# arkworks-rs/circom-compat

Hardware: AMD Instinct MI355X
Metric: Groth16 constraints/sec (BN254) (higher is better)
Workload: dtype int32x9 (29-bit limbs of 254-bit Montgomery integers); 1 GPU; synthetic squaring-chain R1CS, 2^22-2 constraints, BN254, full prove (witness map + 4 G1 MSM + 1 G2 MSM + finalize), trapdoor key minted on GPU; log2_domain=22, num_constraints=4194302, n_vars=4194304, parallelism=single-gpu

## Files before the change

### circom_compat_amd/csrc/api.hip

```cpp
#include "../../include/g16_amd.h"

#include <stddef.h>
#include <stdlib.h>

#include <algorithm>
#include <mutex>

#include "ctx.h"

using namespace g16;

static_assert(offsetof(g16::ProofSums, B1) == sizeof(g16::G1XYZZ29) && offsetof(g16::ProofSums, L) == 2 * sizeof(g16::G1XYZZ29),
              "ProofSums must keep A, B1, L adjacent (batched reduction writes them as an array)");
static_assert(G16_PARTIAL_BYTES == g16::FIN_PARTIAL_BYTES, "partial record size out of sync");

namespace {
std::mutex g_err_mu;
std::string g_create_error;
}


namespace {

g16_status fail(g16_ctx* ctx, g16_status code, const std::string& msg) {
  if (ctx) ctx->err = msg;
  else {
    std::lock_guard<std::mutex> g(g_err_mu);
    g_create_error = msg;
  }
  return code;
}

template <class Fn>
g16_status guarded(g16_ctx* ctx, Fn fn) {
  try {
    if (ctx) G16_HIP(hipSetDevice(ctx->device));
    return fn();
  } catch (const HipError& e) {
    return fail(ctx, G16_ERR_HIP, e.what());
  } catch (const std::bad_alloc&) {
    return fail(ctx, G16_ERR_INTERNAL, "host allocation failed");
  } catch (const std::exception& e) {
    const bool dom = std::string(e.what()).find("PolynomialDegreeTooLarge") != std::string::npos;
    return fail(ctx, dom ? G16_ERR_DOMAIN_TOO_LARGE : G16_ERR_INTERNAL, e.what());
  }
}

void shard(uint32_t len, int rank, int world, uint32_t* lo, uint32_t* hi) {
  *lo = (uint32_t)((uint64_t)len * rank / world);
  *hi = (uint32_t)((uint64_t)len * (rank + 1) / world);
}

int work1_batch(const MsmConfig& cw, uint32_t wr, bool sharded) {
  return (cw.nb() / wr < (1u << 18) || sharded) ? 3 : 2;
}

size_t msm_state_bytes(const MsmConfig& cw, const MsmConfig& ch, uint32_t lw, uint32_t l_cnt, uint32_t lh,
                       uint32_t wr, bool sharded, bool own_w, bool own_h, bool view_w) {
  size_t b = 0;
  if (view_w) b += MsmSort::view_bytes_for(lw, cw);
  if (own_w) b += (size_t)cw.Pn * ((size_t)lw * (64 * 2 + 128) + (size_t)l_cnt * 64);
  if (own_h) b += (size_t)ch.Pn * lh * 64;
  b += MsmSort::bytes_for(lw, cw) + MsmSort::bytes_for(lh, ch);
  const uint32_t nc_w = ceil_div(cw.B, msm_red_chunk(cw, 1, wr)) * cw.D;
  const uint32_t nc_h = ceil_div(ch.B, msm_red_chunk(ch)) * ch.D;
  const uint32_t slots_w = cw.nb() + cw.max_lanes(), slots_h = ch.nb() + ch.max_lanes();
  b += msm_work_bytes<Fq>(slots_w, nc_w, cw.D, work1_batch(cw, wr, sharded)) + msm_work_bytes<Fq2>(slots_w, nc_w, cw.D, 1) +
       msm_work_bytes<Fq>(slots_h, nc_h, ch.D, 1);
  return b;
}

void plan_msm_configs(const g16_options& o, uint32_t lw, uint32_t l_cnt, uint32_t lh, uint32_t wr, bool sharded,
                      bool own_w, bool own_h, bool view_w, MsmConfig* cw, MsmConfig* ch) {
  if (own_w) *cw = msm_make_config(lw ? lw : 1, o.window_bits, o.planes);
  if (own_h) *ch = msm_make_config(lh ? lh : 1, o.window_bits, o.planes);
  if (o.planes > 0) return;
  size_t fr = 0, tot = 0;
  if (hipMemGetInfo(&fr, &tot) != hipSuccess) return;
  const size_t margin = std::min(((size_t)2 << 30) + fr / 50, fr / 4);
  const size_t budget = fr - margin;
  if (msm_state_bytes(*cw, *ch, lw, l_cnt, lh, wr, sharded, own_w, own_h, view_w) <= budget) return;
  auto layouts = [&](const MsmConfig& full, uint32_t len, bool own) {
    std::vector<MsmConfig> v{full};
    for (int pn = full.Pn - 1; own && pn >= 1; --pn) {
      const MsmConfig c = msm_make_config(len ? len : 1, o.window_bits, pn);
      if (c.Pn != v.back().Pn) v.push_back(c);
    }
    return v;
  };
  const std::vector<MsmConfig> vw = layouts(*cw, lw, own_w), vh = layouts(*ch, lh, own_h);
  long best = -1;
  size_t best_bytes = 0;
  for (const MsmConfig& a : vw)
    for (const MsmConfig& b : vh) {
      const size_t need = msm_state_bytes(a, b, lw, l_cnt, lh, wr, sharded, own_w, own_h, view_w);
      if (need > budget) continue;
      const long score = 5L * a.D + b.D;
      if (best < 0 || score < best || (score == best && need > best_bytes)) {
        best = score;
        best_bytes = need;
        *cw = a;
        *ch = b;
      }
    }
  if (best < 0) {
    if (!own_w && !own_h)
      throw std::runtime_error("the sort and partial-sum state of this ctx does not fit the device memory that is free (" +
                               std::to_string(fr >> 20) + " MiB)");
    throw std::runtime_error("the proving key does not fit this device's memory even with one plane per point (" +
                             std::to_string(fr >> 20) + " MiB free)");
  }
}

inline bool sched_r5() {
  static const bool v = [] { const char* e = getenv("G16_SCHED_R5"); return e && atoi(e) != 0; }();
  return v;
}

void collect_times(g16_ctx* c) {
  if (c->timer.enabled) c->timer.collect(c->st_ms, c->st_cnt);
}

void accumulate_ab(g16_ctx* c, hipStream_t s, StageTimer* tm, bool fixup = true) {
  if (c->ptsA.stride == 2) {
    msm_accumulate_pair<Fq>(c->sort_w, c->ptsA, c->ptsB1, c->work1, 0, s, tm, fixup);
  } else {
    msm_accumulate<Fq>(c->sort_w, c->ptsA, 0, c->work1, 0, s, tm, fixup);
    msm_accumulate<Fq>(c->sort_w, c->ptsB1, 0, c->work1, 1, s, tm, fixup);
  }
}
void fixup_ab(g16_ctx* c, hipStream_t q) {
  StageTimer* tm = c->timer.enabled ? &c->timer : nullptr;
  if (c->ptsA.stride == 2) {
    msm_fixup_pair<Fq>(c->sort_w, c->ptsA, c->ptsB1, c->work1, 0, q, tm);
  } else {
    msm_fixup<Fq>(c->sort_w, c->ptsA, 0, c->work1, 0, q, tm);
    msm_fixup<Fq>(c->sort_w, c->ptsB1, 0, c->work1, 1, q, tm);
  }
}

void enqueue_witness_sort(g16_ctx* c, const Fr* w_dev) {
  hipStream_t s = c->stream;
  StageTimer* tm = c->timer.enabled ? &c->timer : nullptr;
  int id = tm ? tm->begin(ST_MSM_SORT, s) : -1;
  c->sort_w.run(w_dev + 1 + c->w_lo, c->w_hi - c->w_lo, true, s);
  if (tm) tm->end(id, s);
  if (c->sparse_b) {
    hipStream_t v = c->overlap ? c->red : s;
    G16_HIP(hipEventRecord(c->ev_view, s));
    G16_HIP(hipStreamWaitEvent(v, c->ev_view, 0));
    id = tm ? tm->begin(ST_MSM_SORT, v) : -1;
    c->sort_b.run_view(c->sort_w, c->keep_b, v);
    if (tm) tm->end(id, v);
    G16_HIP(hipEventRecord(c->ev_view, v));
  }
}
void wait_for_b_view(g16_ctx* c, hipStream_t s) {
  if (c->sparse_b) G16_HIP(hipStreamWaitEvent(s, c->ev_view, 0));
}

template <class Hook, class Hook2>
void enqueue_witness_msms(g16_ctx* c, const Fr* w_dev, Hook after_ab, Hook2 after_b2, bool sorted = false) {
  hipStream_t s = c->stream;
  StageTimer* tm = c->timer.enabled ? &c->timer : nullptr;
  ProofSums* S = c->sums_dev.p;
  if (!sorted) enqueue_witness_sort(c, w_dev);
  const uint32_t nb_eff = c->cfg_w.nb() / (c->shard_buckets ? (uint32_t)c->world : 1u);
  const bool small = nb_eff < (1u << 18);
  const uint32_t b2_limit = c->world > 1 ? (1u << 18) : (1u << 16);
  const bool b2_off = c->overlap && nb_eff < b2_limit;
  const bool sharded = c->world > 1 || c->dist_wm;
  const bool mid = (nb_eff >= (1u << 15) && small) || (sharded && nb_eff >= (1u << 15));
  if (mid && c->overlap && c->work1.batch >= 3) {
    hipStream_t q = c->red;
    accumulate_ab(c, s, tm, false);
    G16_HIP(hipEventRecord(c->ev_acc[0], s));
    G16_HIP(hipStreamWaitEvent(q, c->ev_acc[0], 0));
    fixup_ab(c, q);
    msm_reduce<Fq>(c->sort_w, c->work1, 0, 2, &S->A, q, tm, true);
    after_ab(q);
    wait_for_b_view(c, s);
    msm_accumulate<Fq2>(c->sort_for_b(), c->ptsB2, 0, c->work2, 0, s, tm);
    G16_HIP(hipEventRecord(c->ev_acc[1], s));
    G16_HIP(hipStreamWaitEvent(q, c->ev_acc[1], 0));
    msm_reduce<Fq2>(c->sort_for_b(), c->work2, 0, 1, &S->B2, q, tm, true);
    const bool r5 = sched_r5();
    hipStream_t ql = r5 ? q : c->side;
    if (!r5) after_b2();
    msm_accumulate<Fq>(c->sort_w, c->ptsL, c->l_idx_min, c->work1, 2, s, tm, false);
    G16_HIP(hipEventRecord(c->ev_acc[2], s));
    G16_HIP(hipStreamWaitEvent(ql, c->ev_acc[2], 0));
    msm_fixup<Fq>(c->sort_w, c->ptsL, c->l_idx_min, c->work1, 2, ql, tm);
    msm_reduce<Fq>(c->sort_w, c->work1, 2, 1, &S->L, ql, tm, true);
    if (r5) after_b2();
    G16_HIP(hipEventRecord(c->ev_b2, q));
    G16_HIP(hipStreamWaitEvent(c->side, c->ev_b2, 0));
    G16_HIP(hipEventRecord(c->ev_side, c->side));
    return;
  }
  if (small && c->work1.batch >= 3) {
    accumulate_ab(c, s, tm);
    msm_accumulate<Fq>(c->sort_w, c->ptsL, c->l_idx_min, c->work1, 2, s, tm);
    msm_reduce<Fq>(c->sort_w, c->work1, 0, 3, &S->A, s, tm);
    after_ab(s);
  } else {
    accumulate_ab(c, s, tm);
    msm_reduce<Fq>(c->sort_w, c->work1, 0, 2, &S->A, s, tm);
    after_ab(s);
    msm_run<Fq>(c->sort_w, c->ptsL, c->l_idx_min, c->work1, &S->L, s, tm);
  }
  wait_for_b_view(c, s);
  msm_accumulate<Fq2>(c->sort_for_b(), c->ptsB2, 0, c->work2, 0, s, tm);
  hipStream_t rs = b2_off ? c->red : s;
  G16_HIP(hipEventRecord(c->ev_b2, s));
  G16_HIP(hipStreamWaitEvent(rs, c->ev_b2, 0));
  msm_reduce<Fq2>(c->sort_for_b(), c->work2, 0, 1, &S->B2, rs, tm);
  G16_HIP(hipEventRecord(c->ev_b2, rs));
  if (rs != c->red) G16_HIP(hipStreamWaitEvent(c->red, c->ev_b2, 0));
  after_b2();
  G16_HIP(hipEventRecord(c->ev_b2, c->red));
  G16_HIP(hipStreamWaitEvent(c->side, c->ev_b2, 0));
  G16_HIP(hipEventRecord(c->ev_side, c->side));
}

void enqueue_h_msm(g16_ctx* c) {
  hipStream_t s = c->stream;
  StageTimer* tm = c->timer.enabled ? &c->timer : nullptr;
  G16_HIP(hipStreamWaitEvent(s, c->ev_h, 0));
  msm_run<Fq>(c->sort_h, c->ptsH, 0, c->workH, &c->sums_dev.p->H, s, tm);
}

template <class Hook, class Hook2>
void run_msms(g16_ctx* c, const Fr* w_dev, Hook after_ab, Hook2 after_b2) {
  hipStream_t s = c->stream, x = c->overlap ? c->aux : c->stream;
  StageTimer* tm = c->timer.enabled ? &c->timer : nullptr;
  const uint32_t nb_eff = c->cfg_w.nb() / (c->shard_buckets ? (uint32_t)c->world : 1u);
  const bool sort_first = !sched_r5() && c->overlap && c->world == 1 && nb_eff >= (1u << 18) && c->n <= (1u << 24);
  if (sort_first) enqueue_witness_sort(c, w_dev);
  G16_HIP(hipEventRecord(c->ev_w, s));
  G16_HIP(hipStreamWaitEvent(x, c->ev_w, 0));
  int id = tm ? tm->begin(ST_WITNESS_MAP, x) : -1;
  c->wm.run(w_dev, c->h_canon.p, nullptr, x);
  if (tm) tm->end(id, x);
  id = tm ? tm->begin(ST_MSM_SORT, x) : -1;
  c->sort_h.run(c->h_canon.p + c->h_lo, c->h_hi - c->h_lo, false, x);
  if (tm) tm->end(id, x);
  G16_HIP(hipEventRecord(c->ev_h, x));
  enqueue_witness_msms(c, w_dev, after_ab, after_b2, sort_first);
  enqueue_h_msm(c);
}

template <class Hook>
void run_msms(g16_ctx* c, const Fr* w_dev, Hook after_ab) {
  run_msms(c, w_dev, after_ab, [] {});
}

void begin_sharded(g16_ctx* c, const uint64_t r[4], const uint64_t s_[4]) {
// ... 392 lines not shown
                                 (const G1Affine*)key->b_g1_query + 1 + c->w_lo, lw, c->cfg_w, s);
      }
      c->ptsB2.init((const G2Affine*)key->b_g2_query + 1 + c->w_lo, lw, c->cfg_w, s);
      c->l_idx_min = l_first - c->w_lo;
      c->ptsL.init((const G1Affine*)key->l_query + (l_first - c->p), l_cnt, c->cfg_w, s);
    }
    c->sort_h.init(lh, c->cfg_h);
    if (lend_h) {
      borrow(c->ptsH, lender->ptsH);
    } else if (c->dist_wm) {
      std::vector<G1Affine> mine(lh);
      const G1Affine* hq = (const G1Affine*)key->h_query;
      for (uint32_t t = 0; t < lh; ++t)
        memcpy((void*)&mine[t], (const uint8_t*)hq + (size_t)c->wd.global_index(t) * sizeof(G1Affine), sizeof(G1Affine));
      c->ptsH.init(mine.data(), lh, c->cfg_h, s);
      G16_HIP(hipStreamSynchronize(s));
    } else {
      c->ptsH.init((const G1Affine*)key->h_query + c->h_lo, lh, c->cfg_h, s);
    }

    {
      const bool can = c->world == 1 && !c->dist_wm && c->has_key;
      if (o.fixed_tables > 0 && !can)
        throw std::runtime_error("fixed_tables: only a single-device proving ctx (world = 1, no distributed witness map) can use them");
      if (lender && lend_h) {
        if (lender->tbl.active && o.fixed_tables >= 0) c->tbl.borrow(lender->tbl);
        else if (o.fixed_tables > 0) throw std::runtime_error("fixed_tables: the donor has no tables to lend");
      } else if (can && !lender && o.fixed_tables >= 0) {
        const size_t need = tbl_bytes((size_t)2 * lw + l_cnt + lh, lw);
        size_t fr = 0, tot = 0;
        G16_HIP(hipMemGetInfo(&fr, &tot));
        const bool fits = need <= fr / 3;
        const bool small = lw <= TBL_MAX_POINTS && lh <= TBL_MAX_POINTS;
        if (o.fixed_tables > 0 && !fits)
          throw std::runtime_error("fixed_tables: the tables need " + std::to_string(need >> 20) + " MiB, more than a third of the free device memory");
        if (o.fixed_tables > 0 || (small && fits)) {
          try {
            c->tbl.build(key->a_query + 64, key->b_g1_query + 64, key->b_g2_query + 128,
                         key->l_query + (size_t)(l_first - c->p) * 64, key->h_query, lw, l_first - c->w_lo, l_cnt, lh, s);
          } catch (const HipError&) {
            if (o.fixed_tables > 0) throw;
            (void)hipGetLastError();
            (void)hipStreamSynchronize(s);
            c->tbl.release();
          }
        }
      }
    }

    {
      const uint32_t nc_w = ceil_div(c->cfg_w.B, msm_red_chunk(c->cfg_w, 1, wr)) * c->cfg_w.D;
      const uint32_t nc_h = ceil_div(c->cfg_h.B, msm_red_chunk(c->cfg_h)) * c->cfg_h.D;
      const uint32_t slots_w = c->cfg_w.nb() + c->cfg_w.max_lanes(), slots_h = c->cfg_h.nb() + c->cfg_h.max_lanes();
      c->work1.init(slots_w, nc_w, c->cfg_w.D, work1_batch(c->cfg_w, wr, sharded));
      c->workH.init(slots_h, nc_h, c->cfg_h.D, 1);
      c->work2.init(slots_w, nc_w, c->cfg_w.D);
    }

    KeyHeaderDev kh;
    memcpy(&kh.alpha1, key->alpha_g1, 64);
    memcpy(&kh.beta1, key->beta_g1, 64);
    memcpy(&kh.delta1, key->delta_g1, 64);
    memcpy(&kh.a0, key->a_query, 64);
    memcpy(&kh.b1_0, key->b_g1_query, 64);
    memcpy(&kh.beta2, key->beta_g2, 128);
    memcpy(&kh.delta2, key->delta_g2, 128);
    memcpy(&kh.b2_0, key->b_g2_query, 128);
    G16_HIP(hipMemcpyAsync(c->key_dev.p, &kh, sizeof kh, hipMemcpyHostToDevice, s));
    G16_HIP(hipMemsetAsync(c->out_dev.p, 0, c->out_dev.bytes(), s));
    G16_HIP(hipMemsetAsync(c->sums_dev.p, 0, sizeof(ProofSums), s));
    G16_HIP(hipMemsetAsync(c->fin_scr.p, 0, sizeof(FinScratch), s));
    fin_build_tables(c->key_dev.p, c->fin_tab.p, s);
    G16_HIP(hipStreamSynchronize(s));
    return G16_OK;
  });
  if (st != G16_OK) {
    if (err) *err = c->err;
    g16_ctx_destroy(c);
    return st;
  }
  *out = c;
  return G16_OK;
}

}

extern "C" {

g16_status g16_ctx_create(const g16_key_desc* key, const g16_csr* a, const g16_csr* b,
                          uint32_t num_constraints, const g16_options* opt, g16_ctx** out) {
  std::string err;
  const g16_status st = ctx_create_impl(key, a, b, num_constraints, opt, nullptr, out, &err);
  if (st != G16_OK) return fail(nullptr, st, err);
  return G16_OK;
}

g16_status g16_ctx_create_sibling(g16_ctx* donor, const g16_key_desc* key, const g16_csr* a, const g16_csr* b,
                                  uint32_t num_constraints, const g16_options* opt, g16_ctx** out) {
  if (!donor) return fail(nullptr, G16_ERR_INVALID, "null argument");
  g16_options o{};
  if (opt) o = *opt;
  o.device = donor->device;
  o.rank = 0;
  o.world = 1;
  o.dist_wm = 0;
  if (donor->multi || donor->share_from || !donor->has_key)
    return fail(nullptr, G16_ERR_INVALID, "sibling: the donor must be a plain single-device proving ctx that owns its planes");
// ... 707 lines not shown
```

### circom_compat_amd/csrc/common.h

```cpp
#pragma once
#include <stdint.h>
#include <stdio.h>
#include <string.h>

#include <stdexcept>
#include <string>
#include <vector>

#ifdef G16_EMU
#include <tuple>
#define G16_LAUNCH(kern, grid, block, smem, stream, ...)                                  \
  do {                                                                                    \
    auto _g16_args = std::make_tuple(__VA_ARGS__);      \
    emu::launch(dim3(grid), dim3(block), (smem), [&]() {                                  \
      std::apply([](auto&&... _a) { kern(_a...); }, _g16_args);                           \
    });                                                                                   \
  } while (0)
#define G16_DYN_SMEM(name) unsigned char* name = emu::dyn_smem
#else
#include <hip/hip_runtime.h>
#define G16_LAUNCH(kern, grid, block, smem, stream, ...) \
  hipLaunchKernelGGL(kern, dim3(grid), dim3(block), (smem), (stream), __VA_ARGS__)
#define G16_DYN_SMEM(name) extern __shared__ __attribute__((aligned(16))) unsigned char name[]
#endif

#include "ec.h"

namespace g16 {

struct HipError : std::runtime_error {
  int code;
  HipError(int c, const std::string& m) : std::runtime_error(m), code(c) {}
};

#define G16_HIP(expr)                                                                         \
  do {                                                                                        \
    hipError_t _e = (expr);                                                                   \
    if (_e != hipSuccess) {                                                                   \
      char _b[512];                                                                           \
      snprintf(_b, sizeof _b, "%s failed: %s (%s:%d)", #expr, hipGetErrorString(_e), __FILE__, \
               __LINE__);                                                                     \
      throw g16::HipError((int)_e, _b);                                                       \
    }                                                                                         \
  } while (0)

static inline uint32_t ceil_div(uint64_t a, uint64_t b) { return (uint32_t)((a + b - 1) / b); }

template <class T>
struct DevBuf {
  T* p = nullptr;
  size_t n = 0;
  DevBuf() = default;
  DevBuf(const DevBuf&) = delete;
  DevBuf& operator=(const DevBuf&) = delete;
  ~DevBuf() { release(); }
  void alloc(size_t count) {
    release();
    n = count;
    if (count) G16_HIP(hipMalloc((void**)&p, count * sizeof(T)));
  }
  void release() {
    if (p) (void)hipFree(p);
    p = nullptr;
    n = 0;
  }
  size_t bytes() const { return n * sizeof(T); }
};

enum Stage {
  ST_WITNESS_MAP = 0,
  ST_MSM_SORT,
  ST_MSM_ACC_G1,
  ST_MSM_ACC_G2,
  ST_MSM_REDUCE,
  ST_FINALIZE,
  ST_MSM_ACC_G1_PAIR,
// ... 58 lines not shown
```

### circom_compat_amd/csrc/msm.h

```cpp
#pragma once
#include <stdlib.h>
#include "common.h"
#include "ec29.h"

namespace g16 {

constexpr int MSM_ACC_THREADS = 128;
#ifdef G16_EMU
constexpr int MSM_ACC_BLOCKS = 48;
constexpr int MSM_ACC_BLOCKS_G2 = 32;
#else
constexpr int MSM_ACC_BLOCKS = 3072;
constexpr int MSM_ACC_BLOCKS_G2 = 2048;
#endif
constexpr int MSM_MIN_SEG = 8;
constexpr int MSM_SMALL_MULTI = 32;
constexpr int MSM_RED_CHUNK = 16;
constexpr uint32_t MSM_IDX_BITS_WIDE = 27, MSM_IDX_BITS_NARROW = 26;

struct MsmConfig {
  int c = 0;
  int W = 0;
  int Pn = 1;
  int D = 0;
// ... 62 lines not shown
  const uint32_t* range_dev() const { return world > 1 ? range.p : nullptr; }

  void init(uint32_t capacity, const MsmConfig& cfg);
  void set_shard(int rank, int world);
  void run(const void* scalars, uint32_t n, bool mont, hipStream_t stream);
  void init_view(uint32_t capacity, const MsmConfig& cfg);
  void release_view() {
    count.release(); offset.release(); cursor.release(); entries.release(); multi_l.release();
    meta.release(); multi_l2.release(); meta2.release(); scan_tmp.release();
    cap = len = 0;
  }
  void run_view(const MsmSort& src, const uint32_t* keep_bits, hipStream_t stream);
  static size_t view_bytes_for(uint32_t capacity, const MsmConfig& cfg) {
    const uint64_t M = (uint64_t)capacity * cfg.W;
    return (size_t)(M * 4 + 3 * ((uint64_t)cfg.nb() + 1) * 4 + 2 * (M / ((uint64_t)MSM_MIN_SEG * MSM_SMALL_MULTI) + 2) * 4 + 4096);
  }
  size_t device_bytes() const;
  static size_t bytes_for(uint32_t capacity, const MsmConfig& cfg);
};

template <class F>
using MsmAcc = XYZZ29<typename Lazy<F>::type>;

template <class F>
struct MsmPoints {
  MsmConfig cfg;
  uint32_t count = 0;
  DevBuf<Affine<F>> pts;
  const Affine<F>* view = nullptr;
  uint32_t stride = 1, off = 0;
  const Affine<F>* data() const { return view ? view : pts.p; }
  void init(const Affine<F>* host_points, uint32_t count, const MsmConfig& cfg, hipStream_t stream);
  static void init_pair(MsmPoints& a, MsmPoints& b, const Affine<F>* host_a, const Affine<F>* host_b,
                        uint32_t count, const MsmConfig& cfg, hipStream_t stream);
  void init_from_device(const Affine<F>* dev_points, uint32_t count, const MsmConfig& cfg,
                        hipStream_t stream);
};

#ifdef G16_EMU
constexpr uint32_t MSM_FIX_CAP = 512;
#else
constexpr uint32_t MSM_FIX_CAP = 2048;
#endif
struct MsmFixList {
  uint32_t count;
  uint32_t overflow;
  uint32_t slot[MSM_FIX_CAP];
  uint32_t entry[MSM_FIX_CAP];
};

template <class F>
struct MsmWork {
  int batch = 1;
  uint32_t slots = 0, ncontrib = 0;
  int sets = 1;
  DevBuf<MsmAcc<F>> partial;
  DevBuf<MsmAcc<F>> contrib;
  DevBuf<MsmAcc<F>> bsum;
  DevBuf<MsmAcc<F>> wsum;
  DevBuf<MsmFixList> fix;
  void init(uint32_t n_slots, uint32_t n_contrib, int max_sets, int batch = 1);
};

template <class F>
inline size_t msm_work_bytes(uint32_t n_slots, uint32_t n_contrib, int max_sets, int batch) {
  return (size_t)batch * ((size_t)n_slots + n_contrib + (size_t)257 * max_sets) * sizeof(MsmAcc<F>) +
         (size_t)batch * sizeof(MsmFixList);
}

template <class F>
void msm_run(const MsmSort& s, const MsmPoints<F>& pts, uint32_t idx_min, MsmWork<F>& work,
             MsmAcc<F>* out_dev, hipStream_t stream, StageTimer* tm = nullptr);
template <class F>
void msm_accumulate(const MsmSort& s, const MsmPoints<F>& pts, uint32_t idx_min, MsmWork<F>& work,
                    int slot, hipStream_t stream, StageTimer* tm = nullptr, bool fixup = true);
template <class F>
void msm_fixup(const MsmSort& s, const MsmPoints<F>& pts, uint32_t idx_min, MsmWork<F>& work, int slot,
               hipStream_t stream, StageTimer* tm = nullptr);
template <class F>
void msm_accumulate_pair(const MsmSort& s, const MsmPoints<F>& a, const MsmPoints<F>& b,
                         MsmWork<F>& work, int slot, hipStream_t stream, StageTimer* tm = nullptr,
                         bool fixup = true);
template <class F>
void msm_fixup_pair(const MsmSort& s, const MsmPoints<F>& a, const MsmPoints<F>& b, MsmWork<F>& work,
                    int slot, hipStream_t stream, StageTimer* tm = nullptr);
template <class F>
void msm_reduce(const MsmSort& s, MsmWork<F>& work, int first_slot, int nbatch, MsmAcc<F>* out_dev,
                hipStream_t stream, StageTimer* tm = nullptr, bool hidden = false);



}
```

### circom_compat_amd/csrc/msm_curve.inc.h

```cpp
#pragma once
#include <stdlib.h>

#include "msm.h"

namespace g16 {

namespace {

constexpr int ACC_THREADS = MSM_ACC_THREADS;
constexpr uint32_t MSM_EXACT_BLOCKS = 256;

inline bool acc_fast() {
  static const bool v = [] { const char* e = getenv("G16_ACC_FAST"); return !e || atoi(e) != 0; }();
  return v;
}
template <class F>
constexpr bool acc_is_g1() { return sizeof(F) == sizeof(Fq); }
constexpr int COMB_THREADS = 64;
constexpr int SUM_THREADS = 128;

template <class F>
__global__ void __launch_bounds__(128) k_precompute_planes(Affine<F>* pts, uint32_t count, int Pn,
                                                           int shift_bits, uint32_t stride,
                                                           uint32_t off) {
// ... 298 lines not shown
      if (left > (uint32_t)MSM_SMALL_MULTI) left = 1;
      pending = true;
    }
    const bool is_slot = left > 0;
    MsmAcc<F> x = is_slot ? run : acc, y = run;
    if (is_slot) y = partial[first + --left];
    x.add(y);
    if (is_slot) {
      run = x;
    } else {
      acc = x;
      pending = false;
    }
  }
  if (lo != 0 && !run.is_inf()) {
    uint64_t digits = 0;
    uint32_t v = lo;
    int nd = 0;
    for (uint32_t m = (chunks_per_set - 1) * red_chunk; m != 0 || nd == 0; m >>= 2) ++nd;
    ++nd;
    for (int d = 0; d < nd; ++d) {
      uint32_t t = v & 3u;
      v >>= 2;
      if (t == 3u) {
        ++v;
        t = 0u;
      } else {
        ++t;
      }
      digits |= (uint64_t)t << (3 * d);
    }
    contrib[q] = acc;
    MsmAcc<F> run2 = run;
    run2.dbl_in_place();
    MsmAcc<F> m = MsmAcc<F>::infinity();
    for (int d = nd - 1; d >= 0; --d) {
      m.dbl_in_place();
      m.dbl_in_place();
      const uint32_t t = (uint32_t)(digits >> (3 * d)) & 7u;
      if (t != 1u) {
        MsmAcc<F> y = t == 3u ? run2 : run;
        if (t == 0u) y = y.neg();
        m.add(y);
      }
    }
    acc = contrib[q];
    acc.add(m);
  }
  contrib[q] = acc;
}

template <class F>
__global__ void __launch_bounds__(SUM_THREADS)
    k_set_sum(const MsmAcc<F>* __restrict__ in, uint32_t per_set, uint32_t nblk, MsmAcc<F>* out,
              size_t in_stride, size_t out_stride, const uint32_t* __restrict__ range,
              uint32_t red_chunk) {
  G16_DYN_SMEM(smem_raw);
  MsmAcc<F>* sh = reinterpret_cast<MsmAcc<F>*>(smem_raw);
  in += (size_t)blockIdx.y * in_stride;
  out += (size_t)blockIdx.y * out_stride;
  const uint32_t set = blockIdx.x / nblk, blk = blockIdx.x % nblk;
  const MsmAcc<F>* c = in + (size_t)set * per_set;
  uint32_t k_lo = 0, k_hi = per_set;
  if (range) {
    const uint64_t q_lo = range[4] / red_chunk, q_hi = (range[5] + red_chunk - 1) / red_chunk;
    const uint64_t s_lo = (uint64_t)set * per_set, s_hi = s_lo + per_set;
    const uint64_t a = q_lo > s_lo ? q_lo : s_lo, b = q_hi < s_hi ? q_hi : s_hi;
    k_lo = b > a ? (uint32_t)(a - s_lo) : 0u;
    k_hi = b > a ? (uint32_t)(b - s_lo) : 0u;
  }
  MsmAcc<F> acc = MsmAcc<F>::infinity();
  for (uint32_t k = k_lo + blk * SUM_THREADS + threadIdx.x; k < k_hi; k += nblk * SUM_THREADS)
    acc.add(c[k]);
  MsmAcc<F> tot = block_sum<F, SUM_THREADS>(acc, sh);
  if (threadIdx.x == 0) out[blockIdx.x] = tot;
}

template <class F>
__global__ void k_horner(const MsmAcc<F>* wsum, int stride, int D, int c, MsmAcc<F>* out) {
  if (threadIdx.x != 0) return;
  wsum += (size_t)blockIdx.x * stride;
  out += blockIdx.x;
  MsmAcc<F> t = wsum[D - 1];
  for (int d = D - 2; d >= 0; --d) {
    for (int s = 0; s < c; ++s) t.dbl_in_place();
    t.add(wsum[d]);
  }
  out[0] = t;
}

}

template <class F>
void MsmPoints<F>::init_from_device(const Affine<F>* dev_points, uint32_t n, const MsmConfig& c,
                                    hipStream_t stream) {
  cfg = c;
  count = n;
  pts.alloc((size_t)cfg.Pn * (n ? n : 1));
  if (!n) return;
  G16_HIP(hipMemcpyAsync(pts.p, dev_points, (size_t)n * sizeof(Affine<F>), hipMemcpyDeviceToDevice,
                         stream));
  G16_LAUNCH((k_precompute_planes<F>), ceil_div(n, 128), 128, 0, stream, pts.p, n, cfg.Pn,
             cfg.c * cfg.D, 1u, 0u);
}

template <class F>
void MsmPoints<F>::init(const Affine<F>* host_points, uint32_t n, const MsmConfig& c,
                        hipStream_t stream) {
  cfg = c;
  count = n;
  pts.alloc((size_t)cfg.Pn * (n ? n : 1));
  if (!n) return;
  G16_HIP(hipMemcpyAsync(pts.p, host_points, (size_t)n * sizeof(Affine<F>), hipMemcpyHostToDevice,
                         stream));
  G16_LAUNCH((k_precompute_planes<F>), ceil_div(n, 128), 128, 0, stream, pts.p, n, cfg.Pn,
             cfg.c * cfg.D, 1u, 0u);
}

template <class F>
void MsmPoints<F>::init_pair(MsmPoints<F>& a, MsmPoints<F>& b, const Affine<F>* host_a,
                             const Affine<F>* host_b, uint32_t n, const MsmConfig& c,
                             hipStream_t stream) {
  a.cfg = b.cfg = c;
  a.count = b.count = n;
  a.stride = b.stride = 2;
  a.off = 0;
  b.off = 1;
  a.pts.alloc((size_t)2 * c.Pn * (n ? n : 1));
  a.view = nullptr;
  b.view = a.pts.p;
  if (!n) return;
  const size_t rec = sizeof(Affine<F>);
  G16_HIP(hipMemcpy2DAsync(a.pts.p, 2 * rec, host_a, rec, rec, n, hipMemcpyHostToDevice, stream));
  G16_HIP(hipMemcpy2DAsync(a.pts.p + 1, 2 * rec, host_b, rec, rec, n, hipMemcpyHostToDevice, stream));
  for (uint32_t h = 0; h < 2; ++h)
    G16_LAUNCH((k_precompute_planes<F>), ceil_div(n, 128), 128, 0, stream, a.pts.p, n, c.Pn,
               c.c * c.D, 2u, h);
}

template <class F>
void MsmWork<F>::init(uint32_t n_slots, uint32_t n_contrib, int max_sets, int batch_) {
  slots = n_slots ? n_slots : 1;
  ncontrib = n_contrib ? n_contrib : 1;
  sets = max_sets;
  batch = batch_;
  partial.alloc((size_t)batch * slots);
  contrib.alloc((size_t)batch * ncontrib);
  bsum.alloc((size_t)batch * 256 * sets);
  wsum.alloc((size_t)batch * sets);
  fix.alloc((size_t)batch);
  G16_HIP(hipMemset(fix.p, 0, (size_t)batch * sizeof(MsmFixList)));
}

template <class F>
void msm_accumulate(const MsmSort& s, const MsmPoints<F>& P, uint32_t idx_min, MsmWork<F>& work,
                    int slot, hipStream_t stream, StageTimer* tm, bool fixup) {
  const MsmConfig& cfg = s.cfg;
  const uint32_t nb = cfg.nb();
  const int acc_stage = sizeof(F) == sizeof(Fq) ? ST_MSM_ACC_G1 : ST_MSM_ACC_G2;
  if (slot < 0 || slot >= work.batch) throw std::runtime_error("msm_accumulate: bad workspace slot");
  const uint32_t lanes = s.lanes_of(sizeof(F) != sizeof(Fq));
  const uint32_t grid = lanes / ACC_THREADS;
#ifdef G16_DEBUG_GATHER
  static const bool mask_set = [] {
    if (const char* e = getenv("G16_DEBUG_GATHER_MASK")) {
      const uint32_t m = (uint32_t)strtoul(e, nullptr, 0);
      G16_HIP(hipMemcpyToSymbol(HIP_SYMBOL(g_gather_mask), &m, sizeof m));
    }
    return true;
  }();
  (void)mask_set;
#endif
  int id = tm ? tm->begin(acc_stage, stream) : -1;
  MsmAcc<F>* out = work.partial.p + (size_t)slot * work.slots;
  const uint32_t* en = (const uint32_t*)s.entries.p;
  const uint32_t* of = (const uint32_t*)s.offset.p;
  if constexpr (acc_is_g1<F>()) {
    if (acc_fast()) {
      MsmFixList* fix = work.fix.p + slot;
      if (P.stride == 2)
        G16_LAUNCH((k_bucket_accumulate<F, 2, false, true>), grid, ACC_THREADS, 0, stream, P.data() + P.off,
                   P.count, idx_min, cfg.idx_bits, en, of, nb, lanes, out, (size_t)0, fix);
      else
        G16_LAUNCH((k_bucket_accumulate<F, 1, false, true>), grid, ACC_THREADS, 0, stream, P.data(), P.count,
                   idx_min, cfg.idx_bits, en, of, nb, lanes, out, (size_t)0, fix);
      if (tm) tm->end(id, stream);
      if (fixup) msm_fixup<F>(s, P, idx_min, work, slot, stream, tm);
      return;
    }
  }
  if (P.stride == 2)
    G16_LAUNCH((k_bucket_accumulate<F, 2, false, false>), grid, ACC_THREADS, 0, stream, P.data() + P.off,
               P.count, idx_min, cfg.idx_bits, en, of, nb, lanes, out, (size_t)0, (MsmFixList*)nullptr);
  else
    G16_LAUNCH((k_bucket_accumulate<F, 1, false, false>), grid, ACC_THREADS, 0, stream, P.data(), P.count,
               idx_min, cfg.idx_bits, en, of, nb, lanes, out, (size_t)0, (MsmFixList*)nullptr);
  if (tm) tm->end(id, stream);
}

template <class F>
void msm_fixup(const MsmSort& s, const MsmPoints<F>& P, uint32_t idx_min, MsmWork<F>& work, int slot,
               hipStream_t stream, StageTimer* tm) {
// ... 24 lines not shown
  }
}

template <class F>
void msm_accumulate_pair(const MsmSort& s, const MsmPoints<F>& A, const MsmPoints<F>& B,
                         MsmWork<F>& work, int slot, hipStream_t stream, StageTimer* tm, bool fixup) {
  const MsmConfig& cfg = s.cfg;
  const uint32_t nb = cfg.nb();
  const int acc_stage = ST_MSM_ACC_G1_PAIR;
  if (slot < 0 || slot + 2 > work.batch) throw std::runtime_error("msm_accumulate_pair: bad workspace slot");
  if (A.stride != 2 || B.stride != 2 || A.data() != B.data() || A.off != 0 || B.off != 1 ||
      A.count != B.count)
    throw std::runtime_error("msm_accumulate_pair: the queries are not an interleaved pair");
  const uint32_t grid = cfg.lanes / (ACC_THREADS / 2);
  int id = tm ? tm->begin(acc_stage, stream) : -1;
  const uint32_t* en = (const uint32_t*)s.entries.p;
  const uint32_t* of = (const uint32_t*)s.offset.p;
  MsmAcc<F>* out = work.partial.p + (size_t)slot * work.slots;
  if constexpr (sizeof(F) == sizeof(Fq)) {
    if (acc_fast()) {
      G16_LAUNCH((k_bucket_accumulate<F, 2, true, true>), grid, ACC_THREADS, 0, stream, A.data(), A.count, 0u,
                 cfg.idx_bits, en, of, nb, cfg.lanes, out, (size_t)work.slots, work.fix.p + slot);
      if (tm) tm->end(id, stream);
      if (fixup) msm_fixup_pair<F>(s, A, B, work, slot, stream, tm);
      return;
    }
  }
  G16_LAUNCH((k_bucket_accumulate<F, 2, true, false>), grid, ACC_THREADS, 0, stream, A.data(), A.count, 0u,
             cfg.idx_bits, en, of, nb, cfg.lanes, out, (size_t)work.slots, (MsmFixList*)nullptr);
  if (tm) tm->end(id, stream);
}

template <class F>
void msm_fixup_pair(const MsmSort& s, const MsmPoints<F>& A, const MsmPoints<F>& B, MsmWork<F>& work,
                    int slot, hipStream_t stream, StageTimer* tm) {
  (void)B;
  if constexpr (sizeof(F) == sizeof(Fq)) {
    if (!acc_fast()) return;
    const int tid = tm ? tm->begin(ST_MSM_FIXUP, stream) : -1;
    const MsmConfig& cfg = s.cfg;
    const uint32_t nb = cfg.nb();
    const uint32_t grid = cfg.lanes / (ACC_THREADS / 2);
    MsmAcc<F>* out = work.partial.p + (size_t)slot * work.slots;
    MsmFixList* fix = work.fix.p + slot;
    const uint32_t grid_x = grid < MSM_EXACT_BLOCKS ? grid : MSM_EXACT_BLOCKS;
    G16_LAUNCH((k_acc_fixup<F, 2>), 1, 256, 0, stream, A.data(), A.count, 0u, cfg.idx_bits, fix, out, (size_t)work.slots);
    G16_LAUNCH((k_bucket_accumulate<F, 2, true, false>), grid_x, ACC_THREADS, 0, stream, A.data(), A.count, 0u,
               cfg.idx_bits, (const uint32_t*)s.entries.p, (const uint32_t*)s.offset.p, nb, cfg.lanes, out,
               (size_t)work.slots, fix);
    if (tm) tm->end(tid, stream);
  }
}

template <class F>
void msm_reduce(const MsmSort& s, MsmWork<F>& work, int first_slot, int nbatch, MsmAcc<F>* out_dev,
                hipStream_t stream, StageTimer* tm, bool hidden) {
  const MsmConfig& cfg = s.cfg;
  const uint32_t nb = cfg.nb();
  if (first_slot < 0 || nbatch < 1 || first_slot + nbatch > work.batch)
    throw std::runtime_error("msm_reduce: bad workspace slots");
  MsmAcc<F>* partial = work.partial.p + (size_t)first_slot * work.slots;
  int id = tm ? tm->begin(ST_MSM_REDUCE, stream) : -1;
  const bool g2 = sizeof(F) != sizeof(Fq);
  const uint32_t lanes = s.lanes_of(g2);
  G16_LAUNCH((k_combine_large<F>), dim3(1024, nbatch), COMB_THREADS, COMB_THREADS * sizeof(MsmAcc<F>),
             stream, s.large_list(g2), s.large_meta(g2),
             (const uint32_t*)s.offset.p, nb, lanes, partial, (size_t)work.slots);
  const uint32_t* rng = s.range_dev();
  const uint32_t red_chunk = msm_red_chunk(cfg, (uint32_t)nbatch, (uint32_t)s.world, hidden);
  const uint32_t cps = ceil_div(cfg.B, red_chunk);
  const uint32_t nchunks = cps * (uint32_t)cfg.D;
  if (nchunks > work.ncontrib) throw std::runtime_error("msm_reduce: contribution buffer too small");
  MsmAcc<F>* contrib = work.contrib.p + (size_t)first_slot * work.ncontrib;
  MsmAcc<F>* bsum = work.bsum.p + (size_t)first_slot * 256 * work.sets;
  MsmAcc<F>* wsum = work.wsum.p + (size_t)first_slot * work.sets;
  G16_LAUNCH((k_bucket_reduce<F>), dim3(ceil_div(nchunks, 64), nbatch), 64, 0, stream,
             (const MsmAcc<F>*)partial, (const uint32_t*)s.offset.p, nb, lanes, cfg.B, red_chunk,
             cps, nchunks, contrib, (size_t)work.slots, rng);
  uint32_t nblk = ceil_div(cps / (uint32_t)s.world, SUM_THREADS * 2);
  if (nblk > 256) nblk = 256;
  if (nblk < 1) nblk = 1;
  G16_LAUNCH((k_set_sum<F>), dim3((uint32_t)cfg.D * nblk, nbatch), SUM_THREADS,
             SUM_THREADS * sizeof(MsmAcc<F>), stream, (const MsmAcc<F>*)contrib, cps, nblk,
             bsum, (size_t)nchunks, (size_t)256 * work.sets, rng, red_chunk);
  G16_LAUNCH((k_set_sum<F>), dim3((uint32_t)cfg.D, nbatch), SUM_THREADS,
             SUM_THREADS * sizeof(MsmAcc<F>), stream, (const MsmAcc<F>*)bsum, nblk, 1u,
             wsum, (size_t)256 * work.sets, (size_t)work.sets, (const uint32_t*)nullptr, 1u);
  G16_LAUNCH((k_horner<F>), nbatch, 64, 0, stream, (const MsmAcc<F>*)wsum, work.sets, cfg.D,
             cfg.c, out_dev);
  if (tm) tm->end(id, stream);
}

template <class F>
void msm_run(const MsmSort& s, const MsmPoints<F>& P, uint32_t idx_min, MsmWork<F>& work,
             MsmAcc<F>* out_dev, hipStream_t stream, StageTimer* tm) {
  msm_accumulate<F>(s, P, idx_min, work, 0, stream, tm);
  msm_reduce<F>(s, work, 0, 1, out_dev, stream, tm);
}

}
```

### circom_compat_amd/csrc/msm_g1.hip

```cpp
#include "msm_curve.inc.h"
namespace g16 {
template struct MsmPoints<Fq>;
template struct MsmWork<Fq>;
template void msm_run<Fq>(const MsmSort&, const MsmPoints<Fq>&, uint32_t, MsmWork<Fq>&, MsmAcc<Fq>*,
                          hipStream_t, StageTimer*);
template void msm_accumulate<Fq>(const MsmSort&, const MsmPoints<Fq>&, uint32_t, MsmWork<Fq>&, int,
                                 hipStream_t, StageTimer*, bool);
template void msm_fixup<Fq>(const MsmSort&, const MsmPoints<Fq>&, uint32_t, MsmWork<Fq>&, int, hipStream_t, StageTimer*);
template void msm_accumulate_pair<Fq>(const MsmSort&, const MsmPoints<Fq>&, const MsmPoints<Fq>&,
                                      MsmWork<Fq>&, int, hipStream_t, StageTimer*, bool);
template void msm_fixup_pair<Fq>(const MsmSort&, const MsmPoints<Fq>&, const MsmPoints<Fq>&, MsmWork<Fq>&, int,
                                 hipStream_t, StageTimer*);
template void msm_reduce<Fq>(const MsmSort&, MsmWork<Fq>&, int, int, MsmAcc<Fq>*, hipStream_t,
                             StageTimer*, bool);
}
```

### circom_compat_amd/csrc/msm_g2.hip

```cpp
#include "msm_curve.inc.h"
namespace g16 {
template struct MsmPoints<Fq2>;
template struct MsmWork<Fq2>;
template void msm_run<Fq2>(const MsmSort&, const MsmPoints<Fq2>&, uint32_t, MsmWork<Fq2>&,
                           MsmAcc<Fq2>*, hipStream_t, StageTimer*);
template void msm_accumulate<Fq2>(const MsmSort&, const MsmPoints<Fq2>&, uint32_t, MsmWork<Fq2>&, int,
                                 hipStream_t, StageTimer*, bool);
template void msm_fixup<Fq2>(const MsmSort&, const MsmPoints<Fq2>&, uint32_t, MsmWork<Fq2>&, int, hipStream_t, StageTimer*);
template void msm_reduce<Fq2>(const MsmSort&, MsmWork<Fq2>&, int, int, MsmAcc<Fq2>*, hipStream_t,
                             StageTimer*, bool);
}
```

Baseline: 117.1 million constraints/s.

## Split MSM reduction into wide and tail phases, offload tails to side streams

Splits msm_reduce into a wide bucket-reduce phase and a narrow tail (set sums plus Horner). For large single-GPU runs, the tails for A/B1, L and B2 run on side streams so the main stream can start the next accumulate sooner. It also fuses the two k_set_sum launches into one by using an atomic ticket, so the last block of each set does the final sum. A third scratch slot is added so the L reduction does not overwrite the A/B1 scratch while that tail may still be running. The cost is extra workspace memory and the risk of races through the shared contrib buffers between streams.

```diff
diff --git a/circom_compat_amd/csrc/api.hip b/circom_compat_amd/csrc/api.hip
--- a/circom_compat_amd/csrc/api.hip
+++ b/circom_compat_amd/csrc/api.hip
@@ -54,6 +54,7 @@
 int work1_batch(const MsmConfig& cw, uint32_t wr, bool sharded) {
   return (cw.nb() / wr < (1u << 18) || sharded) ? 3 : 2;
 }
+constexpr int WORK1_SCRATCH = 3;
 
 size_t msm_state_bytes(const MsmConfig& cw, const MsmConfig& ch, uint32_t lw, uint32_t l_cnt, uint32_t lh,
                        uint32_t wr, bool sharded, bool own_w, bool own_h, bool view_w) {
@@ -65,7 +66,7 @@
   const uint32_t nc_w = ceil_div(cw.B, msm_red_chunk(cw, 1, wr)) * cw.D;
   const uint32_t nc_h = ceil_div(ch.B, msm_red_chunk(ch)) * ch.D;
   const uint32_t slots_w = cw.nb() + cw.max_lanes(), slots_h = ch.nb() + ch.max_lanes();
-  b += msm_work_bytes<Fq>(slots_w, nc_w, cw.D, work1_batch(cw, wr, sharded)) + msm_work_bytes<Fq2>(slots_w, nc_w, cw.D, 1) +
+  b += msm_work_bytes<Fq>(slots_w, nc_w, cw.D, work1_batch(cw, wr, sharded), WORK1_SCRATCH) + msm_work_bytes<Fq2>(slots_w, nc_w, cw.D, 1) +
        msm_work_bytes<Fq>(slots_h, nc_h, ch.D, 1);
   return b;
 }
@@ -171,6 +172,7 @@
   const bool b2_off = c->overlap && nb_eff < b2_limit;
   const bool sharded = c->world > 1 || c->dist_wm;
   const bool mid = (nb_eff >= (1u << 15) && small) || (sharded && nb_eff >= (1u << 15));
+  const bool tails_off = !small && !sharded && c->world == 1 && c->overlap;
   if (mid && c->overlap && c->work1.batch >= 3) {
     hipStream_t q = c->red;
     accumulate_ab(c, s, tm, false);
@@ -203,6 +205,30 @@
     msm_accumulate<Fq>(c->sort_w, c->ptsL, c->l_idx_min, c->work1, 2, s, tm);
     msm_reduce<Fq>(c->sort_w, c->work1, 0, 3, &S->A, s, tm);
     after_ab(s);
+  } else if (tails_off) {
+    hipStream_t sd = c->side;
+    accumulate_ab(c, s, tm);
+    msm_reduce_wide<Fq>(c->sort_w, c->work1, 0, 2, s, tm);
+    G16_HIP(hipEventRecord(c->ev_acc[0], s));
+    G16_HIP(hipStreamWaitEvent(sd, c->ev_acc[0], 0));
+    msm_reduce_tail<Fq>(c->sort_w, c->work1, 0, 2, &S->A, sd, tm);
+    after_ab(sd);
+    msm_accumulate<Fq>(c->sort_w, c->ptsL, c->l_idx_min, c->work1, 0, s, tm);
+    msm_reduce_wide<Fq>(c->sort_w, c->work1, 0, 1, s, tm, false, 2);
+    G16_HIP(hipEventRecord(c->ev_acc[2], s));
+    G16_HIP(hipStreamWaitEvent(sd, c->ev_acc[2], 0));
+    msm_reduce_tail<Fq>(c->sort_w, c->work1, 0, 1, &S->L, sd, tm, false, 2);
+    wait_for_b_view(c, s);
+    msm_accumulate<Fq2>(c->sort_for_b(), c->ptsB2, 0, c->work2, 0, s, tm);
+    msm_reduce_wide<Fq2>(c->sort_for_b(), c->work2, 0, 1, s, tm);
+    G16_HIP(hipEventRecord(c->ev_b2, s));
+    G16_HIP(hipStreamWaitEvent(c->red, c->ev_b2, 0));
+    msm_reduce_tail<Fq2>(c->sort_for_b(), c->work2, 0, 1, &S->B2, c->red, tm);
+    after_b2();
+    G16_HIP(hipEventRecord(c->ev_b2, c->red));
+    G16_HIP(hipStreamWaitEvent(sd, c->ev_b2, 0));
+    G16_HIP(hipEventRecord(c->ev_side, sd));
+    return;
   } else {
     accumulate_ab(c, s, tm);
     msm_reduce<Fq>(c->sort_w, c->work1, 0, 2, &S->A, s, tm);
@@ -701,7 +727,7 @@
       const uint32_t nc_w = ceil_div(c->cfg_w.B, msm_red_chunk(c->cfg_w, 1, wr)) * c->cfg_w.D;
       const uint32_t nc_h = ceil_div(c->cfg_h.B, msm_red_chunk(c->cfg_h)) * c->cfg_h.D;
       const uint32_t slots_w = c->cfg_w.nb() + c->cfg_w.max_lanes(), slots_h = c->cfg_h.nb() + c->cfg_h.max_lanes();
-      c->work1.init(slots_w, nc_w, c->cfg_w.D, work1_batch(c->cfg_w, wr, sharded));
+      c->work1.init(slots_w, nc_w, c->cfg_w.D, work1_batch(c->cfg_w, wr, sharded), WORK1_SCRATCH);
       c->workH.init(slots_h, nc_h, c->cfg_h.D, 1);
       c->work2.init(slots_w, nc_w, c->cfg_w.D);
     }
diff --git a/circom_compat_amd/csrc/common.h b/circom_compat_amd/csrc/common.h
--- a/circom_compat_amd/csrc/common.h
+++ b/circom_compat_amd/csrc/common.h
@@ -17,11 +17,13 @@
     });                                                                                   \
   } while (0)
 #define G16_DYN_SMEM(name) unsigned char* name = emu::dyn_smem
+#define G16_FENCE() ((void)0)
 #else
 #include <hip/hip_runtime.h>
 #define G16_LAUNCH(kern, grid, block, smem, stream, ...) \
   hipLaunchKernelGGL(kern, dim3(grid), dim3(block), (smem), (stream), __VA_ARGS__)
 #define G16_DYN_SMEM(name) extern __shared__ __attribute__((aligned(16))) unsigned char name[]
+#define G16_FENCE() __threadfence()
 #endif
 
 #include "ec.h"
diff --git a/circom_compat_amd/csrc/msm.h b/circom_compat_amd/csrc/msm.h
--- a/circom_compat_amd/csrc/msm.h
+++ b/circom_compat_amd/csrc/msm.h
@@ -138,20 +138,23 @@
 template <class F>
 struct MsmWork {
   int batch = 1;
+  int scratch = 1;
   uint32_t slots = 0, ncontrib = 0;
   int sets = 1;
   DevBuf<MsmAcc<F>> partial;
   DevBuf<MsmAcc<F>> contrib;
   DevBuf<MsmAcc<F>> bsum;
   DevBuf<MsmAcc<F>> wsum;
+  DevBuf<uint32_t> ticket;
   DevBuf<MsmFixList> fix;
-  void init(uint32_t n_slots, uint32_t n_contrib, int max_sets, int batch = 1);
+  void init(uint32_t n_slots, uint32_t n_contrib, int max_sets, int batch = 1, int scratch_slots = 0);
 };
 
 template <class F>
-inline size_t msm_work_bytes(uint32_t n_slots, uint32_t n_contrib, int max_sets, int batch) {
-  return (size_t)batch * ((size_t)n_slots + n_contrib + (size_t)257 * max_sets) * sizeof(MsmAcc<F>) +
-         (size_t)batch * sizeof(MsmFixList);
+inline size_t msm_work_bytes(uint32_t n_slots, uint32_t n_contrib, int max_sets, int batch, int scratch_slots = 0) {
+  const size_t sc = (size_t)(scratch_slots > batch ? scratch_slots : batch);
+  return ((size_t)batch * n_slots + sc * ((size_t)n_contrib + (size_t)257 * max_sets)) * sizeof(MsmAcc<F>) +
+         (size_t)batch * sizeof(MsmFixList) + sc * (size_t)max_sets * sizeof(uint32_t);
 }
 
 template <class F>
@@ -173,6 +176,12 @@
 template <class F>
 void msm_reduce(const MsmSort& s, MsmWork<F>& work, int first_slot, int nbatch, MsmAcc<F>* out_dev,
                 hipStream_t stream, StageTimer* tm = nullptr, bool hidden = false);
+template <class F>
+void msm_reduce_wide(const MsmSort& s, MsmWork<F>& work, int first_slot, int nbatch, hipStream_t stream,
+                     StageTimer* tm = nullptr, bool hidden = false, int scratch_slot = -1);
+template <class F>
+void msm_reduce_tail(const MsmSort& s, MsmWork<F>& work, int first_slot, int nbatch, MsmAcc<F>* out_dev,
+                     hipStream_t stream, StageTimer* tm = nullptr, bool hidden = false, int scratch_slot = -1);
 
 
 
diff --git a/circom_compat_amd/csrc/msm_curve.inc.h b/circom_compat_amd/csrc/msm_curve.inc.h
--- a/circom_compat_amd/csrc/msm_curve.inc.h
+++ b/circom_compat_amd/csrc/msm_curve.inc.h
@@ -374,13 +374,16 @@
 
 template <class F>
 __global__ void __launch_bounds__(SUM_THREADS)
-    k_set_sum(const MsmAcc<F>* __restrict__ in, uint32_t per_set, uint32_t nblk, MsmAcc<F>* out,
-              size_t in_stride, size_t out_stride, const uint32_t* __restrict__ range,
-              uint32_t red_chunk) {
+    k_set_sum(const MsmAcc<F>* __restrict__ in, uint32_t per_set, uint32_t nblk, MsmAcc<F>* bsum,
+              MsmAcc<F>* wsum, uint32_t* ticket, size_t in_stride, size_t bsum_stride, size_t wsum_stride,
+              const uint32_t* __restrict__ range, uint32_t red_chunk) {
   G16_DYN_SMEM(smem_raw);
   MsmAcc<F>* sh = reinterpret_cast<MsmAcc<F>*>(smem_raw);
+  __shared__ uint32_t last;
   in += (size_t)blockIdx.y * in_stride;
-  out += (size_t)blockIdx.y * out_stride;
+  bsum += (size_t)blockIdx.y * bsum_stride;
+  wsum += (size_t)blockIdx.y * wsum_stride;
+  ticket += (size_t)blockIdx.y * wsum_stride;
   const uint32_t set = blockIdx.x / nblk, blk = blockIdx.x % nblk;
   const MsmAcc<F>* c = in + (size_t)set * per_set;
   uint32_t k_lo = 0, k_hi = per_set;
@@ -395,7 +398,22 @@
   for (uint32_t k = k_lo + blk * SUM_THREADS + threadIdx.x; k < k_hi; k += nblk * SUM_THREADS)
     acc.add(c[k]);
   MsmAcc<F> tot = block_sum<F, SUM_THREADS>(acc, sh);
-  if (threadIdx.x == 0) out[blockIdx.x] = tot;
+  if (threadIdx.x == 0) {
+    bsum[blockIdx.x] = tot;
+    G16_FENCE();
+    last = atomicAdd(ticket + set, 1u) == nblk - 1 ? 1u : 0u;
+  }
+  __syncthreads();
+  if (!last) return;
+  G16_FENCE();
+  const MsmAcc<F>* bs = bsum + (size_t)set * nblk;
+  acc = MsmAcc<F>::infinity();
+  for (uint32_t k = threadIdx.x; k < nblk; k += SUM_THREADS) acc.add(bs[k]);
+  tot = block_sum<F, SUM_THREADS>(acc, sh);
+  if (threadIdx.x == 0) {
+    wsum[set] = tot;
+    ticket[set] = 0u;
+  }
 }
 
 template <class F>
@@ -461,15 +479,18 @@
 }
 
 template <class F>
-void MsmWork<F>::init(uint32_t n_slots, uint32_t n_contrib, int max_sets, int batch_) {
+void MsmWork<F>::init(uint32_t n_slots, uint32_t n_contrib, int max_sets, int batch_, int scratch_slots) {
   slots = n_slots ? n_slots : 1;
   ncontrib = n_contrib ? n_contrib : 1;
   sets = max_sets;
   batch = batch_;
+  scratch = scratch_slots > batch ? scratch_slots : batch;
   partial.alloc((size_t)batch * slots);
-  contrib.alloc((size_t)batch * ncontrib);
-  bsum.alloc((size_t)batch * 256 * sets);
-  wsum.alloc((size_t)batch * sets);
+  contrib.alloc((size_t)scratch * ncontrib);
+  bsum.alloc((size_t)scratch * 256 * sets);
+  wsum.alloc((size_t)scratch * sets);
+  ticket.alloc((size_t)scratch * sets);
+  G16_HIP(hipMemset(ticket.p, 0, (size_t)scratch * sets * sizeof(uint32_t)));
   fix.alloc((size_t)batch);
   G16_HIP(hipMemset(fix.p, 0, (size_t)batch * sizeof(MsmFixList)));
 }
@@ -600,13 +621,36 @@
   }
 }
 
-template <class F>
-void msm_reduce(const MsmSort& s, MsmWork<F>& work, int first_slot, int nbatch, MsmAcc<F>* out_dev,
-                hipStream_t stream, StageTimer* tm, bool hidden) {
+namespace {
+struct RedShape {
+  uint32_t red_chunk, cps, nchunks, nblk;
+};
+template <class F>
+RedShape red_shape(const MsmSort& s, const MsmWork<F>& work, int first_slot, int nbatch, bool hidden,
+                   int scratch_slot) {
+  const MsmConfig& cfg = s.cfg;
+  if (first_slot < 0 || nbatch < 1 || first_slot + nbatch > work.batch || scratch_slot < 0 ||
+      scratch_slot + nbatch > work.scratch)
+    throw std::runtime_error("msm_reduce: bad workspace slots");
+  RedShape r;
+  r.red_chunk = msm_red_chunk(cfg, (uint32_t)nbatch, (uint32_t)s.world, hidden);
+  r.cps = ceil_div(cfg.B, r.red_chunk);
+  r.nchunks = r.cps * (uint32_t)cfg.D;
+  if (r.nchunks > work.ncontrib) throw std::runtime_error("msm_reduce: contribution buffer too small");
+  r.nblk = ceil_div(r.cps / (uint32_t)s.world, SUM_THREADS * 2);
+  if (r.nblk > 256) r.nblk = 256;
+  if (r.nblk < 1) r.nblk = 1;
+  return r;
+}
+}
+
+template <class F>
+void msm_reduce_wide(const MsmSort& s, MsmWork<F>& work, int first_slot, int nbatch, hipStream_t stream,
+                     StageTimer* tm, bool hidden, int scratch_slot) {
   const MsmConfig& cfg = s.cfg;
   const uint32_t nb = cfg.nb();
-  if (first_slot < 0 || nbatch < 1 || first_slot + nbatch > work.batch)
-    throw std::runtime_error("msm_reduce: bad workspace slots");
+  if (scratch_slot < 0) scratch_slot = first_slot;
+  const RedShape r = red_shape(s, work, first_slot, nbatch, hidden, scratch_slot);
   MsmAcc<F>* partial = work.partial.p + (size_t)first_slot * work.slots;
   int id = tm ? tm->begin(ST_MSM_REDUCE, stream) : -1;
   const bool g2 = sizeof(F) != sizeof(Fq);
@@ -614,29 +658,37 @@
   G16_LAUNCH((k_combine_large<F>), dim3(1024, nbatch), COMB_THREADS, COMB_THREADS * sizeof(MsmAcc<F>),
              stream, s.large_list(g2), s.large_meta(g2),
              (const uint32_t*)s.offset.p, nb, lanes, partial, (size_t)work.slots);
-  const uint32_t* rng = s.range_dev();
-  const uint32_t red_chunk = msm_red_chunk(cfg, (uint32_t)nbatch, (uint32_t)s.world, hidden);
-  const uint32_t cps = ceil_div(cfg.B, red_chunk);
-  const uint32_t nchunks = cps * (uint32_t)cfg.D;
-  if (nchunks > work.ncontrib) throw std::runtime_error("msm_reduce: contribution buffer too small");
-  MsmAcc<F>* contrib = work.contrib.p + (size_t)first_slot * work.ncontrib;
-  MsmAcc<F>* bsum = work.bsum.p + (size_t)first_slot * 256 * work.sets;
-  MsmAcc<F>* wsum = work.wsum.p + (size_t)first_slot * work.sets;
-  G16_LAUNCH((k_bucket_reduce<F>), dim3(ceil_div(nchunks, 64), nbatch), 64, 0, stream,
-             (const MsmAcc<F>*)partial, (const uint32_t*)s.offset.p, nb, lanes, cfg.B, red_chunk,
-             cps, nchunks, contrib, (size_t)work.slots, rng);
-  uint32_t nblk = ceil_div(cps / (uint32_t)s.world, SUM_THREADS * 2);
-  if (nblk > 256) nblk = 256;
-  if (nblk < 1) nblk = 1;
-  G16_LAUNCH((k_set_sum<F>), dim3((uint32_t)cfg.D * nblk, nbatch), SUM_THREADS,
-             SUM_THREADS * sizeof(MsmAcc<F>), stream, (const MsmAcc<F>*)contrib, cps, nblk,
-             bsum, (size_t)nchunks, (size_t)256 * work.sets, rng, red_chunk);
-  G16_LAUNCH((k_set_sum<F>), dim3((uint32_t)cfg.D, nbatch), SUM_THREADS,
-             SUM_THREADS * sizeof(MsmAcc<F>), stream, (const MsmAcc<F>*)bsum, nblk, 1u,
-             wsum, (size_t)256 * work.sets, (size_t)work.sets, (const uint32_t*)nullptr, 1u);
+  MsmAcc<F>* contrib = work.contrib.p + (size_t)scratch_slot * work.ncontrib;
+  G16_LAUNCH((k_bucket_reduce<F>), dim3(ceil_div(r.nchunks, 64), nbatch), 64, 0, stream,
+             (const MsmAcc<F>*)partial, (const uint32_t*)s.offset.p, nb, lanes, cfg.B, r.red_chunk,
+             r.cps, r.nchunks, contrib, (size_t)work.slots, s.range_dev());
+  if (tm) tm->end(id, stream);
+}
+
+template <class F>
+void msm_reduce_tail(const MsmSort& s, MsmWork<F>& work, int first_slot, int nbatch, MsmAcc<F>* out_dev,
+                     hipStream_t stream, StageTimer* tm, bool hidden, int scratch_slot) {
+  const MsmConfig& cfg = s.cfg;
+  if (scratch_slot < 0) scratch_slot = first_slot;
+  const RedShape r = red_shape(s, work, first_slot, nbatch, hidden, scratch_slot);
+  int id = tm ? tm->begin(ST_MSM_REDUCE, stream) : -1;
+  const MsmAcc<F>* contrib = work.contrib.p + (size_t)scratch_slot * work.ncontrib;
+  MsmAcc<F>* bsum = work.bsum.p + (size_t)scratch_slot * 256 * work.sets;
+  MsmAcc<F>* wsum = work.wsum.p + (size_t)scratch_slot * work.sets;
+  uint32_t* ticket = work.ticket.p + (size_t)scratch_slot * work.sets;
+  G16_LAUNCH((k_set_sum<F>), dim3((uint32_t)cfg.D * r.nblk, nbatch), SUM_THREADS,
+             SUM_THREADS * sizeof(MsmAcc<F>), stream, contrib, r.cps, r.nblk, bsum, wsum, ticket,
+             (size_t)r.nchunks, (size_t)256 * work.sets, (size_t)work.sets, s.range_dev(), r.red_chunk);
   G16_LAUNCH((k_horner<F>), nbatch, 64, 0, stream, (const MsmAcc<F>*)wsum, work.sets, cfg.D,
              cfg.c, out_dev);
   if (tm) tm->end(id, stream);
+}
+
+template <class F>
+void msm_reduce(const MsmSort& s, MsmWork<F>& work, int first_slot, int nbatch, MsmAcc<F>* out_dev,
+                hipStream_t stream, StageTimer* tm, bool hidden) {
+  msm_reduce_wide<F>(s, work, first_slot, nbatch, stream, tm, hidden);
+  msm_reduce_tail<F>(s, work, first_slot, nbatch, out_dev, stream, tm, hidden);
 }
 
 template <class F>
diff --git a/circom_compat_amd/csrc/msm_g1.hip b/circom_compat_amd/csrc/msm_g1.hip
--- a/circom_compat_amd/csrc/msm_g1.hip
+++ b/circom_compat_amd/csrc/msm_g1.hip
@@ -13,4 +13,7 @@
                                  hipStream_t, StageTimer*);
 template void msm_reduce<Fq>(const MsmSort&, MsmWork<Fq>&, int, int, MsmAcc<Fq>*, hipStream_t,
                              StageTimer*, bool);
+template void msm_reduce_wide<Fq>(const MsmSort&, MsmWork<Fq>&, int, int, hipStream_t, StageTimer*, bool, int);
+template void msm_reduce_tail<Fq>(const MsmSort&, MsmWork<Fq>&, int, int, MsmAcc<Fq>*, hipStream_t,
+                                  StageTimer*, bool, int);
 }
diff --git a/circom_compat_amd/csrc/msm_g2.hip b/circom_compat_amd/csrc/msm_g2.hip
--- a/circom_compat_amd/csrc/msm_g2.hip
+++ b/circom_compat_amd/csrc/msm_g2.hip
@@ -9,4 +9,7 @@
 template void msm_fixup<Fq2>(const MsmSort&, const MsmPoints<Fq2>&, uint32_t, MsmWork<Fq2>&, int, hipStream_t, StageTimer*);
 template void msm_reduce<Fq2>(const MsmSort&, MsmWork<Fq2>&, int, int, MsmAcc<Fq2>*, hipStream_t,
                              StageTimer*, bool);
+template void msm_reduce_wide<Fq2>(const MsmSort&, MsmWork<Fq2>&, int, int, hipStream_t, StageTimer*, bool, int);
+template void msm_reduce_tail<Fq2>(const MsmSort&, MsmWork<Fq2>&, int, int, MsmAcc<Fq2>*, hipStream_t,
+                                  StageTimer*, bool, int);
 }
```

Measured after the change: 117.7 million constraints/s, median of 6. Within noise of the previous version (+0.5%).
